# double125/MADTP

Hardware: AMD Instinct MI355X
Metric: images/sec forward, BLIP-base NLVR2 p=0.5 b64; pruned-token index match (higher is better)
Workload: dtype bf16

## Files before the change

### madtp_amd/csrc/attention.hip

```cpp
#include "common.h"
#include "internal.h"
#include <map>
#include <mutex>
#include <stdlib.h>

namespace {

struct AttnArgs {
    const char* q; const char* k; const char* v; char* out; const float* mask;
    float* colsum; float* p0; float* onorm;
    int B, H, Nq, Nk, ldq, ldk, ldv, ldo, nrt;
    float scale;
    const int* kvidx;
    const char* q2; const char* k2; const char* v2; char* out2; const float* mask2; int pair;
    const float* mask_qk; int ld_mqk;
    unsigned* hm_ws; int* hm_tick;
    int kvb;
    float* o_part;
    const int32_t* n_dev;
    int dev_q_only;
    int split_dim; int* range_flag;
};
#define ATTN_DEV_DIMS(a)                                   \
    if ((a).n_dev) {                                       \
// ... 373 lines not shown
#pragma unroll
        for (int t = 0; t < NT; ++t) {
            const int off = (16 * t + l16) * PITCH + g * 16;
            const f16x8 kh0 = *(const f16x8*)(K0 + off), kh1 = *(const f16x8*)(K0 + off + 64);
            const f16x8 kl0 = *(const f16x8*)(K1 + off), kl1 = *(const f16x8*)(K1 + off + 64);
            const f32x4 z = (f32x4){0.f, 0.f, 0.f, 0.f};
            f32x4 hi = __builtin_amdgcn_mfma_f32_16x16x32_f16(kh0, qh[0], z, 0, 0, 0);
            hi = __builtin_amdgcn_mfma_f32_16x16x32_f16(kh1, qh[1], hi, 0, 0, 0);
            f32x4 lo = __builtin_amdgcn_mfma_f32_16x16x32_f16(kh0, ql[0], z, 0, 0, 0);
            lo = __builtin_amdgcn_mfma_f32_16x16x32_f16(kh1, ql[1], lo, 0, 0, 0);
            lo = __builtin_amdgcn_mfma_f32_16x16x32_f16(kl0, qh[0], lo, 0, 0, 0);
            lo = __builtin_amdgcn_mfma_f32_16x16x32_f16(kl1, qh[1], lo, 0, 0, 0);
#pragma unroll
            for (int r = 0; r < 4; ++r) sc[t][r] = fmaf(lo[r], LO, hi[r]);
        }

        float m = -INFINITY;
#pragma unroll
        for (int t = 0; t < NT; ++t)
#pragma unroll
            for (int r = 0; r < 4; ++r) {
                const float v = __fadd_rn(__fmul_rn(sc[t][r], a.scale), mk[t][r]);
                sc[t][r] = v;
                m = fmaxf(m, v);
            }
        m = rows4_max(m);
        float sum = 0.f;
#pragma unroll
        for (int t = 0; t < NT; ++t)
#pragma unroll
            for (int r = 0; r < 4; ++r) {
                const float p = expf(sc[t][r] - m);
                sc[t][r] = p;
                sum += p;
            }
        sum = rows4_sum(sum);
#pragma unroll
        for (int t = 0; t < NT; ++t)
#pragma unroll
            for (int r = 0; r < 4; ++r) {
                const float p = sc[t][r] / sum;
                sc[t][r] = p;
                if constexpr (SCORES) pmax[t][r] = fmaxf(pmax[t][r], p);
            }
        if constexpr (SCORES) {
            if (i0 == 0 && l16 == 0) {
                float* dst = a.p0 + ((size_t)b * a.H + h) * a.Nk;
#pragma unroll
                for (int t = 0; t < NT; ++t)
#pragma unroll
                    for (int r = 0; r < 4; ++r) {
                        const int j = 16 * t + 4 * g + r;
                        if (j < a.Nk) dst[j] = sc[t][r];
                    }
            }
        }

        f32x4 oh[4], ol[4];
#pragma unroll
        for (int dt = 0; dt < 4; ++dt) { oh[dt] = (f32x4){0.f, 0.f, 0.f, 0.f}; ol[dt] = (f32x4){0.f, 0.f, 0.f, 0.f}; }
#pragma unroll
        for (int c = 0; c < NC; ++c) {
            const f32x4 t1 = (2 * c + 1 < NT) ? sc[2 * c + 1 < NT ? 2 * c + 1 : 0] : (f32x4){0.f, 0.f, 0.f, 0.f};
            u32x4 pp0, pp1;
            split_f16x8(sc[2 * c], t1, pp0, pp1);
            const f16x8 ph = __builtin_bit_cast(f16x8, pp0), pl = __builtin_bit_cast(f16x8, pp1);
            const int voff = (32 * c + 4 * g + (l16 >> 2)) * PITCH + 8 * (l16 & 3);
#pragma unroll
            for (int dt = 0; dt < 4; ++dt) {
                const bf16x8 vh = cat_bf16x4(lds_read_tr16(V0 + voff + dt * 32), lds_read_tr16(V0 + voff + 16 * PITCH + dt * 32));
                const bf16x8 vl = cat_bf16x4(lds_read_tr16(V1 + voff + dt * 32), lds_read_tr16(V1 + voff + 16 * PITCH + dt * 32));
                oh[dt] = __builtin_amdgcn_mfma_f32_16x16x32_f16(__builtin_bit_cast(f16x8, vh), ph, oh[dt], 0, 0, 0);
                ol[dt] = __builtin_amdgcn_mfma_f32_16x16x32_f16(__builtin_bit_cast(f16x8, vh), pl, ol[dt], 0, 0, 0);
                ol[dt] = __builtin_amdgcn_mfma_f32_16x16x32_f16(__builtin_bit_cast(f16x8, vl), ph, ol[dt], 0, 0, 0);
            }
        }

        {
            const int i = i0 + l16;
            f32x4 o[4];
            float n2 = 0.f;
#pragma unroll
            for (int dt = 0; dt < 4; ++dt)
#pragma unroll
                for (int r = 0; r < 4; ++r) {
                    o[dt][r] = fmaf(ol[dt][r], LO, oh[dt][r]);
                    n2 += o[dt][r] * o[dt][r];
                }
            if constexpr (SCORES) n2 = rows4_sum(n2);
            if (i < a.Nq) {
                if (a.split_dim) {
                    _Float16* prow = (_Float16*)a.out + ((size_t)b * a.Nq + i) * a.ldo + h * 64 + 4 * g;
                    bool bad = false;
#pragma unroll
                    for (int dt = 0; dt < 4; ++dt) {
                        f16x4 ph_, pl_;
                        split_f16x4(o[dt], ph_, pl_);
                        *(f16x4*)(prow + dt * 16) = ph_;
                        *(f16x4*)(prow + a.split_dim + dt * 16) = pl_;
                        bad |= f16_range_bad(o[dt]);
                    }
                    f16_range_raise(a.range_flag, bad);
                } else {
                    float* orow = (float*)(a.out + (((size_t)b * a.Nq + i) * a.ldo + h * 64) * 4) + 4 * g;
#pragma unroll
                    for (int dt = 0; dt < 4; ++dt) *(f32x4*)(orow + dt * 16) = o[dt];
                }
                if constexpr (SCORES)
                    if (g == 0) a.onorm[((size_t)b * a.H + h) * a.Nq + i] = sqrtf(n2);
            }
        }
    }

    if constexpr (SCORES) {
        if (gridDim.z == 2) {
            const size_t slot = ((size_t)b * gridDim.x + blockIdx.x) * 4 + wave;
            unsigned* mine = a.hm_ws + ((slot * 2 + blockIdx.z) * (2 * HM_MAX_NT)) * 64 + lane;
#pragma unroll
            for (int t = 0; t < NT; ++t)
#pragma unroll
                for (int r = 0; r < 4; ++r)
                    __hip_atomic_store(mine + (4 * t + r) * 64, __float_as_uint(pmax[t][r]), __ATOMIC_RELAXED, __HIP_MEMORY_SCOPE_AGENT);
            asm volatile("s_waitcnt vmcnt(0)" ::: "memory");
            int old = 0;
            if (lane == 0) old = __hip_atomic_fetch_add(a.hm_tick + slot, 1, __ATOMIC_RELAXED, __HIP_MEMORY_SCOPE_AGENT);
            old = __builtin_amdgcn_readfirstlane(old);
            if (old == 0) return;
            if (lane == 0) __hip_atomic_store(a.hm_tick + slot, 0, __ATOMIC_RELAXED, __HIP_MEMORY_SCOPE_AGENT);
            const unsigned* theirs = a.hm_ws + ((slot * 2 + (1 - blockIdx.z)) * (2 * HM_MAX_NT)) * 64 + lane;
#pragma unroll
            for (int t = 0; t < NT; ++t)
#pragma unroll
                for (int r = 0; r < 4; ++r)
                    pmax[t][r] = fmaxf(pmax[t][r], __uint_as_float(__hip_atomic_load(theirs + (4 * t + r) * 64, __ATOMIC_RELAXED,
                                                                                      __HIP_MEMORY_SCOPE_AGENT)));
        }
        if (active) {
            const int i = i0 + l16;
            const bool valid = i >= 1 && i < a.Nq;
            float* dst = a.colsum + ((size_t)b * a.nrt + rt) * a.Nk;
#pragma unroll
            for (int t = 0; t < NT; ++t)
#pragma unroll
                for (int r = 0; r < 4; ++r) {
                    const float v = row16_sum(valid ? pmax[t][r] : 0.f);
                    const int j = 16 * t + 4 * g + r;
                    if (l16 == 0 && j < a.Nk) dst[j] = v;
                }
        }
    }
}

#ifdef MADTP_TS_TIMING
__device__ long long g_attn_dbg[8];
#define AT_MARK(i) do { if (threadIdx.x == 0 && blockIdx.x == 0 && blockIdx.y == 0 && it == 2) { __builtin_amdgcn_s_waitcnt(0); g_attn_dbg[i] = wall_clock64(); } } while (0)
#else
#define AT_MARK(i)
#endif
template <int NT, bool SCORES, int HS, int RB = 1, bool F16 = false>
__global__ __launch_bounds__(256 * HS * RB, (HS == 1 && RB == 1) ? 2 : 1) void attn_bf16_kernel(AttnArgs a) {
    ATTN_DEV_DIMS(a)
    static_assert(HS == 1 || RB == 1, "head-parity split and two row blocks are alternatives");
    constexpr int NKP = NT * 16;
    constexpr int NC = (NT + 1) / 2;
    constexpr int VR = NC * 32;
    constexpr int STAGE = (NKP + VR) * 128;
    extern __shared__ __attribute__((aligned(16))) char smem[];

    const int tid = threadIdx.x, lane = tid & 63;
    const int wave8 = __builtin_amdgcn_readfirstlane(tid >> 6);
    const int wave = wave8 & 3;
    const int hp = HS == 2 ? wave8 >> 2 : 0;
    const int rb = RB == 2 ? wave8 >> 2 : 0;
    constexpr int NSW = 4 * RB;
    const int swave = RB == 2 ? wave8 : wave;
    char* const ring = smem + hp * 2 * STAGE;
    const int l16 = lane & 15, g = lane >> 4;
    int b = blockIdx.y;
    if (a.pair && b >= a.B) {
        b -= a.B;
        a.q = a.q2; a.k = a.k2; a.v = a.v2; a.out = a.out2; a.mask = a.mask2;
    }
    const int bkv = a.kvidx ? a.kvidx[b] : b;
    const int rt = (blockIdx.x * RB + rb) * 4 + wave;
    const int i0 = rt * 16;
    const bool active = i0 < a.Nq;
    const int irow = min(i0 + l16, a.Nq - 1);

    f32x4 pmax[NT];
    if constexpr (SCORES) {
#pragma unroll
        for (int t = 0; t < NT; ++t) pmax[t] = (f32x4){0.f, 0.f, 0.f, 0.f};
    }
    f32x4 mk[NT];
#pragma unroll
    for (int t = 0; t < NT; ++t)
#pragma unroll
        for (int r = 0; r < 4; ++r) {
            const int j = 16 * t + 4 * g + r;
            mk[t][r] = j < a.Nk ? (a.mask ? a.mask[(size_t)b * a.Nk + j] : 0.f) : -INFINITY;
            if (a.mask_qk && j < a.Nk) mk[t][r] += a.mask_qk[(size_t)irow * a.ld_mqk + j];
            mk[t][r] *= 1.44269504088896341f;
        }
    const float c2 = a.scale * 1.44269504088896341f;

    const int sub = lane >> 3, pos = lane & 7;
    constexpr int NDMA = ((NKP + VR) / 8 + NSW - 1) / NSW;
    const char* srcb[NDMA];
#pragma unroll
    for (int i = 0; i < NDMA; ++i) {
        const int grp = swave + NSW * i;
        const bool is_v = grp >= NKP / 8;
        int row = (is_v ? grp - NKP / 8 : grp) * 8 + sub;
        const int chunk = is_v ? (pos ^ (((row >> 1) & 3) << 1)) : (pos ^ (row & 7));
        row = row < a.Nk ? row : a.Nk - 1;
        srcb[i] = (is_v ? a.v + ((size_t)bkv * a.kvb + row) * a.ldv * 2 : a.k + ((size_t)bkv * a.kvb + row) * a.ldk * 2) + chunk * 16;
    }
    auto stage_head = [&](int h, int st) {
        char* base = ring + st * STAGE;
#pragma unroll
        for (int i = 0; i < NDMA; ++i) {
            const int grp = swave + NSW * i;
            if (grp < (NKP + VR) / 8)
                __builtin_amdgcn_global_load_lds(GLOBAL_PTR(srcb[i] + h * 128), LDS_PTR(base + grp * 1024), 16, 0, 0);
        }
    };
    const char* qbase = a.q + ((size_t)b * a.Nq + irow) * a.ldq * 2 + g * 16;
    auto load_q = [&](int h, bf16x8 (&qq)[2]) {
        const char* qp = qbase + h * 128;
        qq[0] = *(const bf16x8*)qp;
        qq[1] = *(const bf16x8*)(qp + 64);
    };
    int st = 0;
    const int hstep = gridDim.z * HS;
    const int hfirst = blockIdx.z * HS + hp;
    const int niter = (a.H - (int)blockIdx.z * HS + hstep - 1) / hstep;
    bf16x8 qn[2];
    if (hfirst < a.H) {
        stage_head(hfirst, 0);
        load_q(hfirst, qn);
    }
    for (int it = 0; it < niter; ++it, st ^= 1) {
        const int h = hfirst + it * hstep;
        bf16x8 q[2] = {qn[0], qn[1]};
        AT_MARK(0);
        __syncthreads();
        AT_MARK(1);
        if (h + hstep < a.H) {
            stage_head(h + hstep, st ^ 1);
            load_q(h + hstep, qn);
        }
        if (!active || h >= a.H) continue;
        AT_MARK(2);
        const char* Ks = ring + st * STAGE;
        const char* Vs = Ks + NKP * 128;

        f32x4 sc[NT];
#pragma unroll
        for (int t = 0; t < NT; ++t) {
            const int row = 16 * t + l16;
            const bf16x8 k0 = *(const bf16x8*)(Ks + row * 128 + (((0 + g) ^ (row & 7)) << 4));
            const bf16x8 k1 = *(const bf16x8*)(Ks + row * 128 + (((4 + g) ^ (row & 7)) << 4));
            f32x4 acc = (f32x4){0.f, 0.f, 0.f, 0.f};
            acc = mfma_lp<F16>(k0, q[0], acc, 0, 0, 0);
            sc[t] = mfma_lp<F16>(k1, q[1], acc, 0, 0, 0);
        }
        AT_MARK(3);
        float m = -INFINITY;
#pragma unroll
        for (int t = 0; t < NT; ++t)
#pragma unroll
            for (int r = 0; r < 4; ++r) {
                const float v = fmaf(sc[t][r], c2, mk[t][r]);
                sc[t][r] = v;
                m = fmaxf(m, v);
            }
        m = rows4_max(m);
        float sum = 0.f;
#pragma unroll
        for (int t = 0; t < NT; ++t)
#pragma unroll
            for (int r = 0; r < 4; ++r) {
                const float p = __builtin_amdgcn_exp2f(sc[t][r] - m);
                sc[t][r] = p;
                sum += p;
            }
        sum = rows4_sum(sum);
        const float inv = __builtin_amdgcn_rcpf(sum);
#pragma unroll
        for (int t = 0; t < NT; ++t) {
            sc[t] *= inv;
            if constexpr (SCORES) {
#pragma unroll
                for (int r = 0; r < 4; ++r) pmax[t][r] = fmaxf(pmax[t][r], sc[t][r]);
            }
        }
        if constexpr (SCORES) {
            if (i0 == 0) {
                if (l16 == 0) {
                    float* dst = a.p0 + ((size_t)b * a.H + h) * a.Nk;
#pragma unroll
                    for (int t = 0; t < NT; ++t)
#pragma unroll
                        for (int r = 0; r < 4; ++r) {
                            const int j = 16 * t + 4 * g + r;
                            if (j < a.Nk) dst[j] = sc[t][r];
                        }
                }
            }
        }
        AT_MARK(4);
        f32x4 o[4];
#pragma unroll
        for (int dt = 0; dt < 4; ++dt) o[dt] = (f32x4){0.f, 0.f, 0.f, 0.f};
#pragma unroll
        for (int c = 0; c < NC; ++c) {
            const f32x4 hi = (2 * c + 1 < NT) ? sc[2 * c + 1 < NT ? 2 * c + 1 : 0] : (f32x4){0.f, 0.f, 0.f, 0.f};
            const bf16x8 pa = pack_lp8<F16>(sc[2 * c], hi);
            const int vrow = 32 * c + 4 * g + (l16 >> 2);
            const int vkey = ((vrow >> 1) & 3) << 1;
            const char* vr = Vs + vrow * 128 + 8 * (l16 & 1);
#pragma unroll
            for (int dt = 0; dt < 4; ++dt) {
                const int p = ((2 * dt + ((l16 & 3) >> 1)) ^ vkey) << 4;
                const bf16x8 vb = cat_bf16x4(lds_read_tr16(vr + p), lds_read_tr16(vr + 16 * 128 + p));
                o[dt] = mfma_lp<F16>(vb, pa, o[dt], 0, 0, 0);
            }
        }
        AT_MARK(5);
        {
            const int i = i0 + l16;
            float n2 = 0.f;
#pragma unroll
            for (int dt = 0; dt < 4; ++dt)
#pragma unroll
                for (int r = 0; r < 4; ++r) n2 += o[dt][r] * o[dt][r];
            if constexpr (SCORES) {
                n2 = rows4_sum(n2);
            }
            if (i < a.Nq) {
                bf16_t* orow = (bf16_t*)(a.out + (((size_t)b * a.Nq + i) * a.ldo + h * 64) * 2) + 4 * g;
#pragma unroll
                for (int dt = 0; dt < 4; ++dt) *(bf16x4*)(orow + dt * 16) = pack_lp4<F16>(o[dt]);
                if constexpr (SCORES)
                    if (g == 0) a.onorm[((size_t)b * a.H + h) * a.Nq + i] = sqrtf(n2);
            }
        }
        AT_MARK(6);
    }

    if constexpr (SCORES && HS == 2) {
        f32x4* xch = (f32x4*)smem;
        __syncthreads();
        if (hp == 1)
#pragma unroll
            for (int t = 0; t < NT; ++t) xch[(wave * NT + t) * 64 + lane] = pmax[t];
        __syncthreads();
        if (hp == 1) return;
#pragma unroll
        for (int t = 0; t < NT; ++t) {
            const f32x4 o = xch[(wave * NT + t) * 64 + lane];
#pragma unroll
            for (int r = 0; r < 4; ++r) pmax[t][r] = fmaxf(pmax[t][r], o[r]);
        }
    }
    if constexpr (SCORES) {
        if (active) {
            const int i = i0 + l16;
            const bool valid = i >= 1 && i < a.Nq;
            float* dst = a.colsum + ((size_t)b * a.nrt + rt) * a.Nk;
#pragma unroll
            for (int t = 0; t < NT; ++t)
#pragma unroll
                for (int r = 0; r < 4; ++r) {
                    const float v = row16_sum(valid ? pmax[t][r] : 0.f);
                    const int j = 16 * t + 4 * g + r;
                    if (l16 == 0 && j < a.Nk) dst[j] = v;
                }
        }
    }
}

constexpr int SMALL_NW = 12;
template <bool F16>
__global__ __launch_bounds__(64 * SMALL_NW, 1) void attn_bf16_small_kernel(AttnArgs a) {
    __shared__ __attribute__((aligned(16))) char vbuf[SMALL_NW][32 * 128];
    __shared__ float pm[SMALL_NW][2][2][64][4];
    const int tid = threadIdx.x, lane = tid & 63;
    const int wave = __builtin_amdgcn_readfirstlane(tid >> 6);
    const int l16 = lane & 15, g = lane >> 4;
    const int b = blockIdx.x;
    const int N = a.Nk;
    char* Vs = vbuf[wave];
    f32x4 pmax[2][2];
#pragma unroll
    for (int rt = 0; rt < 2; ++rt)
#pragma unroll
        for (int t = 0; t < 2; ++t) pmax[rt][t] = (f32x4){0.f, 0.f, 0.f, 0.f};
    const int nrt = (N + 15) / 16;
    f32x4 mk[2];
#pragma unroll
    for (int t = 0; t < 2; ++t)
#pragma unroll
        for (int r = 0; r < 4; ++r) {
            const int j = 16 * t + 4 * g + r;
            mk[t][r] = (j < N ? (a.mask ? a.mask[(size_t)b * N + j] : 0.f) : -INFINITY) * 1.44269504088896341f;
        }
    const float c2 = a.scale * 1.44269504088896341f;

    for (int h = wave; h < a.H; h += SMALL_NW) {
        {
            const int sub = lane >> 3, pos = lane & 7;
#pragma unroll
            for (int grp = 0; grp < 4; ++grp) {
                int row = grp * 8 + sub;
                const int chunk = pos ^ (((row >> 1) & 3) << 1);
                row = row < N ? row : N - 1;
                *(bf16x8*)(Vs + grp * 1024 + lane * 16) =
                    *(const bf16x8*)(a.v + (((size_t)b * N + row) * a.ldv + h * 64) * 2 + chunk * 16);
            }
        }
        bf16x8 kf[2][2];
#pragma unroll
        for (int t = 0; t < 2; ++t) {
            const int j = min(16 * t + l16, N - 1);
            const char* kp = a.k + (((size_t)b * N + j) * a.ldk + h * 64) * 2 + g * 16;
            kf[t][0] = *(const bf16x8*)kp;
            kf[t][1] = *(const bf16x8*)(kp + 64);
        }
#pragma unroll
        for (int rt = 0; rt < 2; ++rt) {
            if (rt >= nrt) break;
            const int i0 = rt * 16;
            const int irow = min(i0 + l16, N - 1);
            const char* qp = a.q + (((size_t)b * N + irow) * a.ldq + h * 64) * 2 + g * 16;
            const bf16x8 q0 = *(const bf16x8*)qp, q1 = *(const bf16x8*)(qp + 64);
            f32x4 sc[2];
            float m = -INFINITY;
#pragma unroll
            for (int t = 0; t < 2; ++t) {
                f32x4 acc = (f32x4){0.f, 0.f, 0.f, 0.f};
                acc = mfma_lp<F16>(kf[t][0], q0, acc, 0, 0, 0);
                acc = mfma_lp<F16>(kf[t][1], q1, acc, 0, 0, 0);
#pragma unroll
                for (int r = 0; r < 4; ++r) {
                    const float v = fmaf(acc[r], c2, mk[t][r]);
                    acc[r] = v;
                    m = fmaxf(m, v);
                }
                sc[t] = acc;
            }
            m = rows4_max(m);
            float sum = 0.f;
#pragma unroll
            for (int t = 0; t < 2; ++t)
#pragma unroll
                for (int r = 0; r < 4; ++r) { sc[t][r] = __builtin_amdgcn_exp2f(sc[t][r] - m); sum += sc[t][r]; }
            sum = rows4_sum(sum);
            const float inv = __builtin_amdgcn_rcpf(sum);
#pragma unroll
            for (int t = 0; t < 2; ++t) {
                sc[t] *= inv;
#pragma unroll
                for (int r = 0; r < 4; ++r) pmax[rt][t][r] = fmaxf(pmax[rt][t][r], sc[t][r]);
            }
            if (i0 == 0) if (l16 == 0) {
                float* dst = a.p0 + ((size_t)b * a.H + h) * N;
#pragma unroll
                for (int t = 0; t < 2; ++t)
#pragma unroll
                    for (int r = 0; r < 4; ++r) {
                        const int j = 16 * t + 4 * g + r;
                        if (j < N) dst[j] = sc[t][r];
                    }
            }
            const bf16x8 pa = pack_lp8<F16>(sc[0], sc[1]);
            const int vrow = 4 * g + (l16 >> 2);
            const int vkey = ((vrow >> 1) & 3) << 1;
            const char* vr = Vs + vrow * 128 + 8 * (l16 & 1);
            f32x4 o[4];
            float n2 = 0.f;
#pragma unroll
            for (int dt = 0; dt < 4; ++dt) {
                const int p = ((2 * dt + ((l16 & 3) >> 1)) ^ vkey) << 4;
                const bf16x8 vb = cat_bf16x4(lds_read_tr16(vr + p), lds_read_tr16(vr + 16 * 128 + p));
                o[dt] = mfma_lp<F16>(vb, pa, (f32x4){0.f, 0.f, 0.f, 0.f}, 0, 0, 0);
#pragma unroll
                for (int r = 0; r < 4; ++r) n2 += o[dt][r] * o[dt][r];
            }
            n2 = rows4_sum(n2);
            const int i = i0 + l16;
            if (i < N) {
                bf16_t* orow = (bf16_t*)(a.out + (((size_t)b * N + i) * a.ldo + h * 64) * 2) + 4 * g;
#pragma unroll
                for (int dt = 0; dt < 4; ++dt) *(bf16x4*)(orow + dt * 16) = pack_lp4<F16>(o[dt]);
                if (g == 0) a.onorm[((size_t)b * a.H + h) * N + i] = sqrtf(n2);
            }
        }
    }
#pragma unroll
    for (int rt = 0; rt < 2; ++rt)
#pragma unroll
        for (int t = 0; t < 2; ++t)
#pragma unroll
            for (int r = 0; r < 4; ++r) pm[wave][rt][t][lane][r] = pmax[rt][t][r];
    __syncthreads();
    if (wave < nrt) {
        const int rt = wave, i = rt * 16 + l16;
        const bool valid = i >= 1 && i < N;
        float* dst = a.colsum + ((size_t)b * a.nrt + rt) * N;
#pragma unroll
        for (int t = 0; t < 2; ++t)
#pragma unroll
            for (int r = 0; r < 4; ++r) {
                float v = pm[0][rt][t][lane][r];
#pragma unroll
                for (int w = 1; w < SMALL_NW; ++w) v = fmaxf(v, pm[w][rt][t][lane][r]);
                v = row16_sum(valid ? v : 0.f);
                const int j = 16 * t + 4 * g + r;
                if (l16 == 0 && j < N) dst[j] = v;
            }
    }
}

template <int NT, bool SCORES, bool F16>
int launch_attn_bf16(const AttnArgs& a, hipStream_t s) {
    constexpr int NC = (NT + 1) / 2;
    constexpr int HS = (SCORES && NT <= 8) ? 2 : 1;
    constexpr int RB = (SCORES && NT > 8) ? 2 : 1;
    const size_t lds = (size_t)2 * HS * (NT * 16 + NC * 32) * 128;
    MADTP_ENSURE_MAX_LDS((attn_bf16_kernel<NT, SCORES, HS, RB, F16>), lds);
    int gz = 1;
    size_t lds_used = lds;
    if (!SCORES) {
        const int wgs = ((a.Nq + 63) / 64) * a.B;
        gz = wgs >= 512 ? 1 : a.H;
        if (gz == a.H) lds_used = lds / 2;
    }
    hipLaunchKernelGGL((attn_bf16_kernel<NT, SCORES, HS, RB, F16>), dim3((a.Nq + 64 * RB - 1) / (64 * RB), (!SCORES && a.pair) ? 2 * a.B : a.B, gz),
                       dim3(256 * HS * RB), lds_used, s, a);
    MADTP_LAUNCH_CHECK();
    return 0;
}

template <bool SCORES, bool F16 = false>
int dispatch_nt_bf16(const AttnArgs& a, hipStream_t s) {
    const int nt = (a.Nk + 15) / 16;
    if (nt <= 4) return launch_attn_bf16<4, SCORES, F16>(a, s);
    if (nt <= 6) return launch_attn_bf16<6, SCORES, F16>(a, s);
    if (nt <= 8) return launch_attn_bf16<8, SCORES, F16>(a, s);
    if (nt <= 10) return launch_attn_bf16<10, SCORES, F16>(a, s);
    if (nt <= 12) return launch_attn_bf16<12, SCORES, F16>(a, s);
    if (nt <= 13) return launch_attn_bf16<13, SCORES, F16>(a, s);
    if (nt <= 16) return launch_attn_bf16<16, SCORES, F16>(a, s);
    return MADTP_E_SHAPE;
}

template <typename T, int NCH, bool SCORES>
__global__ __launch_bounds__(256, 1) void attn_large_kernel(AttnArgs a) {
    constexpr int ESZ = sizeof(T);
    constexpr int RB = 64 * ESZ + 16;
    constexpr int CPR = 64 * ESZ / 16;
    constexpr int CK = 128;
    constexpr int NT = NCH * 8;
    extern __shared__ __attribute__((aligned(16))) char smem[];
    char* Ks = smem;
    char* Vs = smem + CK * RB;

    const int tid = threadIdx.x, lane = tid & 63, wave = tid >> 6;
    const int l16 = lane & 15, g = lane >> 4;
    const int b = blockIdx.y;
    const int bkv = a.kvidx ? a.kvidx[b] : b;
    const int rt = blockIdx.x * 4 + wave;
    const int i0 = rt * 16;
    const bool active = i0 < a.Nq;
    const int irow = min(i0 + l16, a.Nq - 1);

    f32x4 pmax[SCORES ? NT : 1];
    if constexpr (SCORES) {
#pragma unroll
        for (int t = 0; t < NT; ++t) pmax[t] = (f32x4){0.f, 0.f, 0.f, 0.f};
    }

    auto stage = [&](int h, int c, bool with_v) {
        for (int idx = tid; idx < CK * CPR; idx += 256) {
            const int row = idx / CPR, ch = idx % CPR, j = c * CK + row;
            uint4 kv = make_uint4(0, 0, 0, 0), vv = make_uint4(0, 0, 0, 0);
            if (j < a.Nk) {
                const size_t grow = (size_t)bkv * a.kvb + j;
                kv = *(const uint4*)(a.k + (grow * a.ldk + h * 64) * ESZ + ch * 16);
                if (with_v) vv = *(const uint4*)(a.v + (grow * a.ldv + h * 64) * ESZ + ch * 16);
            }
            *(uint4*)(Ks + row * RB + ch * 16) = kv;
            if (with_v) *(uint4*)(Vs + row * RB + ch * 16) = vv;
        }
    };
    auto scores = [&](int c, const f32x4 (&q)[4], f32x4 (&sc)[8]) {
#pragma unroll
        for (int t = 0; t < 8; ++t) sc[t] = (f32x4){0.f, 0.f, 0.f, 0.f};
#pragma unroll
        for (int s = 0; s < 4; ++s) {
            f32x4 kf[8];
#pragma unroll
            for (int t = 0; t < 8; ++t) kf[t] = load4<T>(Ks + (16 * t + l16) * RB + (4 * s + g) * 4 * ESZ);
#pragma unroll
            for (int e = 0; e < 4; ++e)
#pragma unroll
                for (int t = 0; t < 8; ++t) sc[t] = __builtin_amdgcn_mfma_f32_16x16x4f32(kf[t][e], q[s][e], sc[t], 0, 0, 0);
        }
#pragma unroll
        for (int t = 0; t < 8; ++t)
#pragma unroll
            for (int r = 0; r < 4; ++r) {
                const int j = c * CK + 16 * t + 4 * g + r;
                float v = sc[t][r] * a.scale;
                if (a.mask && j < a.Nk) v += a.mask[(size_t)b * a.Nk + j];
                sc[t][r] = j < a.Nk ? v : -INFINITY;
            }
    };

    for (int h = blockIdx.z; h < a.H; h += gridDim.z) {
        f32x4 q[4];
        {
            const char* qp = a.q + (((size_t)b * a.Nq + irow) * a.ldq + h * 64) * ESZ;
#pragma unroll
            for (int s = 0; s < 4; ++s) q[s] = load4<T>(qp + (4 * s + g) * 4 * ESZ);
        }
        float m = -INFINITY, l = 0.f;
        for (int c = 0; c < NCH; ++c) {
            if (c * CK >= a.Nk) break;
            __syncthreads();
            stage(h, c, false);
            __syncthreads();
            if (!active) continue;
            f32x4 sc[8];
            scores(c, q, sc);
            float cm = -INFINITY;
#pragma unroll
            for (int t = 0; t < 8; ++t)
#pragma unroll
                for (int r = 0; r < 4; ++r) cm = fmaxf(cm, sc[t][r]);
            cm = rows4_max(cm);
            const float mn = fmaxf(m, cm);
            float cs = 0.f;
#pragma unroll
            for (int t = 0; t < 8; ++t)
#pragma unroll
                for (int r = 0; r < 4; ++r) cs += expf(sc[t][r] - mn);
            cs = rows4_sum(cs);
            l = l * expf(m - mn) + cs;
            m = mn;
        }
        f32x4 o[4];
#pragma unroll
        for (int dt = 0; dt < 4; ++dt) o[dt] = (f32x4){0.f, 0.f, 0.f, 0.f};
#pragma unroll
        for (int c = 0; c < NCH; ++c) {
            if (c * CK < a.Nk) {
                __syncthreads();
                stage(h, c, true);
                __syncthreads();
                if (active) {
                    f32x4 sc[8];
                    scores(c, q, sc);
#pragma unroll
                    for (int t = 0; t < 8; ++t) {
#pragma unroll
                        for (int r = 0; r < 4; ++r) {
                            const float p = expf(sc[t][r] - m) / l;
                            sc[t][r] = p;
                            if constexpr (SCORES) pmax[c * 8 + t][r] = fmaxf(pmax[c * 8 + t][r], p);
                        }
                    }
                    if constexpr (SCORES) {
                        if (i0 + l16 == 0) {
                            float* dst = a.p0 + ((size_t)b * a.H + h) * a.Nk;
#pragma unroll
                            for (int t = 0; t < 8; ++t)
#pragma unroll
                                for (int r = 0; r < 4; ++r) {
                                    const int j = c * CK + 16 * t + 4 * g + r;
                                    if (j < a.Nk) dst[j] = sc[t][r];
                                }
// ... 906 lines not shown
}
int madtp_i_attention_mask(const void* q, const void* k, const void* v, void* out, const float* add_mask, float* colsum_part, float* p0,
                           float* onorm, int B, int H, int N, int ldq, int ldk, int ldv, int ldo, float scale, int io_dtype,
                           const int32_t* n_dev, void* stream) {
    if (N > 256) return MADTP_E_SHAPE;
    return madtp_i_attention_launch(q, k, v, nullptr, out, add_mask, nullptr, 0, colsum_part, p0, onorm, B, H, N, N, ldq, ldk, ldv, ldo, scale,
                                    io_dtype, 0, stream, n_dev);
}
int madtp_i_attention_cached(const void* q, const void* k, const void* v, int kv_block_rows, void* out, int B, int H, int Nq, int Nk,
                             int ldq, int ldk, int ldv, int ldo, float scale, int io_dtype, void* stream) {
    return madtp_i_attention_launch(q, k, v, nullptr, out, nullptr, nullptr, 0, nullptr, nullptr, nullptr, B, H, Nq, Nk, ldq, ldk, ldv, ldo, scale,
                                    io_dtype, 0, stream, nullptr, 0, kv_block_rows);
}
int madtp_i_attention_cross(const void* q, const void* k, const void* v, const int32_t* kv_batch_index, void* out, const float* add_mask,
                            int B, int H, int Nq_max, int Nk, int ldq, int ldk, int ldv, int ldo, float scale, int io_dtype,
                            const int32_t* nq_dev, void* stream) {
    if (Nk > 256 || Nq_max > 256) return MADTP_E_SHAPE;
    return madtp_i_attention_launch(q, k, v, kv_batch_index, out, add_mask, nullptr, 0, nullptr, nullptr, nullptr, B, H, Nq_max, Nk, ldq, ldk,
                                    ldv, ldo, scale, io_dtype, 0, stream, nq_dev, 1);
}

extern "C" int madtp_attention_indexed(const void* q, const void* k, const void* v, const int32_t* kv_batch_index, void* out,
                                       const float* add_mask, float* colsum_part, float* p0, float* onorm, int B, int H,
                                       int Nq, int Nk, int ldq, int ldk, int ldv, int ldo, float scale, int io_dtype,
                                       void* stream) {
    return madtp_i_attention_launch(q, k, v, kv_batch_index, out, add_mask, nullptr, 0, colsum_part, p0, onorm, B, H, Nq, Nk, ldq, ldk,
                                    ldv, ldo, scale, io_dtype, 0, stream);
}

extern "C" int madtp_attention_qk_mask(const void* q, const void* k, const void* v, void* out, const float* add_mask,
                                       const float* mask_qk, int ld_mask_qk, float* colsum_part, float* p0, float* onorm, int B,
                                       int H, int Nq, int Nk, int ldq, int ldk, int ldv, int ldo, float scale, int io_dtype,
                                       void* stream) {
    return madtp_i_attention_launch(q, k, v, nullptr, out, add_mask, mask_qk, ld_mask_qk, colsum_part, p0, onorm, B, H, Nq, Nk, ldq, ldk,
                                    ldv, ldo, scale, io_dtype, 0, stream);
}

bool madtp_internal_attn_f16s_enabled() {
    static const int f16s_env = env_int("MADTP_ATTN_F16S", 1);
    return f16s_env != 0;
}

int madtp_i_attention_launch(const void* q, const void* k, const void* v, const int32_t* kv_batch_index, void* out,
                             const float* add_mask, const float* mask_qk, int ld_mask_qk, float* colsum_part, float* p0,
                             float* onorm, int B, int H, int Nq, int Nk, int ldq, int ldk, int ldv, int ldo, float scale,
                             int io_dtype, int split_req, void* stream, const int32_t* n_dev, int dev_q_only, int kv_block_rows) {
    if (!q || !k || !v || !out || B <= 0 || H <= 0 || Nq <= 0 || Nk <= 0) return MADTP_E_BADARG;
    if (mask_qk && (ld_mask_qk < Nk || Nk > 256)) return MADTP_E_SHAPE;
    if (split_req < 0) split_req = 0;
    if (kv_block_rows && (kv_block_rows < Nk || Nk > 256 || colsum_part)) return MADTP_E_SHAPE;
    if (kv_batch_index && colsum_part) return MADTP_E_BADARG;
    if (io_dtype != MADTP_F32 && io_dtype != MADTP_BF16 && io_dtype != MADTP_F16S && io_dtype != MADTP_F16) return MADTP_E_DTYPE;
    bool f16s = io_dtype == MADTP_F16S;
    const bool f16 = io_dtype == MADTP_F16;
    int split_dim = 0;
    if (f16s) {
        f16s = madtp_internal_attn_f16s_enabled();
        io_dtype = MADTP_F32;
        split_dim = f16s ? split_req : 0;
        if (split_req && !f16s) return MADTP_E_BADARG;
    } else if (split_req) {
        return MADTP_E_BADARG;
    }
    if (colsum_part && (!p0 || !onorm || Nq != Nk)) return MADTP_E_BADARG;
    const int esz = (io_dtype == MADTP_BF16 || f16) ? 2 : 4;
    if (!aligned16(q) || !aligned16(k) || !aligned16(v) || (ldq * esz) % 16 || (ldk * esz) % 16 || (ldv * esz) % 16)
        return MADTP_E_ALIGN;
    if (Nk > 1024) return MADTP_E_SHAPE;
    AttnArgs a;
    a.q = (const char*)q; a.k = (const char*)k; a.v = (const char*)v; a.out = (char*)out; a.mask = add_mask;
    a.colsum = colsum_part; a.p0 = p0; a.onorm = onorm;
    a.B = B; a.H = H; a.Nq = Nq; a.Nk = Nk; a.ldq = ldq; a.ldk = ldk; a.ldv = ldv; a.ldo = ldo;
    a.nrt = (Nq + 15) / 16;
    a.scale = scale;
    a.kvidx = kv_batch_index;
    a.pair = 0; a.q2 = a.k2 = a.v2 = nullptr; a.out2 = nullptr; a.mask2 = nullptr; a.hm_ws = nullptr; a.hm_tick = nullptr; a.o_part = nullptr;
    a.mask_qk = mask_qk; a.ld_mqk = ld_mask_qk;
    a.n_dev = n_dev; a.dev_q_only = dev_q_only;
    a.kvb = kv_block_rows ? kv_block_rows : Nk;
    a.split_dim = split_dim; a.range_flag = split_dim ? madtp_internal_range_flag() : nullptr;
    hipStream_t s = (hipStream_t)stream;
    const bool scores = colsum_part != nullptr;
    if (split_dim) {
        if ((ldo % 4) || (split_dim % 4) || ((uintptr_t)out & 7)) return MADTP_E_ALIGN;
        if (Nk > 256) return scores ? dispatch_large_f16s<true>(a, s) : dispatch_large_f16s<false>(a, s);
        return scores ? dispatch_nt_f16s<true>(a, s) : dispatch_nt_f16s<false>(a, s);
    }
    if (Nk > 256) {
        if (f16s && (ldo * 4) % 16 == 0 && aligned16(out))
            return scores ? dispatch_large_f16s<true>(a, s) : dispatch_large_f16s<false>(a, s);
        if (io_dtype == MADTP_F32) return scores ? dispatch_large<float, true>(a, s) : dispatch_large<float, false>(a, s);
        static const int large_env = env_int("MADTP_ATTN_LARGE_F32", 0);
        if (f16) return scores ? dispatch_bf16_large<true, true>(a, s) : dispatch_bf16_large<false, true>(a, s);
        if (large_env) return scores ? dispatch_large<bf16_t, true>(a, s) : dispatch_large<bf16_t, false>(a, s);
        return scores ? dispatch_bf16_large<true>(a, s) : dispatch_bf16_large<false>(a, s);
    }
    if (f16s && (ldo * 4) % 16 == 0 && aligned16(out))
        return scores ? dispatch_nt_f16s<true>(a, s) : dispatch_nt_f16s<false>(a, s);
    if (io_dtype == MADTP_F32) return scores ? dispatch_nt<float, true>(a, s) : dispatch_nt<float, false>(a, s);
    if ((ldk * 2) % 16 || (ldv * 2) % 16) return MADTP_E_ALIGN;
    if (scores && Nk <= 32 && !mask_qk && !n_dev) {
        if (f16) hipLaunchKernelGGL(attn_bf16_small_kernel<true>, dim3(B), dim3(64 * SMALL_NW), 0, s, a);
        else hipLaunchKernelGGL(attn_bf16_small_kernel<false>, dim3(B), dim3(64 * SMALL_NW), 0, s, a);
        MADTP_LAUNCH_CHECK();
        return 0;
    }
    if (f16) return scores ? dispatch_nt_bf16<true, true>(a, s) : dispatch_nt_bf16<false, true>(a, s);
    return scores ? dispatch_nt_bf16<true>(a, s) : dispatch_nt_bf16<false>(a, s);
}

extern "C" int madtp_attention_pair(const void* q0, const void* q1, const void* k0, const void* k1, const void* v0, const void* v1,
                                    const int32_t* kv_batch_index, void* out0, void* out1, const float* add_mask0,
                                    const float* add_mask1, int B, int H, int Nq, int Nk, int ldq, int ldk, int ldv, int ldo,
                                    float scale, int io_dtype, void* stream) {
    return madtp_i_attention_pair(q0, q1, k0, k1, v0, v1, kv_batch_index, out0, out1, add_mask0, add_mask1, B, H, Nq, Nk, ldq, ldk, ldv,
                                  ldo, scale, io_dtype, 0, nullptr, stream);
}
int madtp_i_attention_pair(const void* q0, const void* q1, const void* k0, const void* k1, const void* v0, const void* v1,
                           const int32_t* kv_batch_index, void* out0, void* out1, const float* add_mask0, const float* add_mask1, int B,
                           int H, int Nq, int Nk, int ldq, int ldk, int ldv, int ldo, float scale, int io_dtype, int split_dim,
                           const int32_t* nq_dev, void* stream) {
    if (nq_dev && (Nk > 256 || Nq > 256)) return MADTP_E_SHAPE;
    if (!q0 || !q1 || !k0 || !k1 || !v0 || !v1 || !out0 || !out1 || B <= 0 || H <= 0 || Nq <= 0 || Nk <= 0) return MADTP_E_BADARG;
    static const int pair_env = env_int("MADTP_ATTN_PAIR", 1);
    const bool one = pair_env && (io_dtype == MADTP_BF16 || io_dtype == MADTP_F16) && Nk <= 256 && (!add_mask0) == (!add_mask1) && aligned16(q0) &&
                     aligned16(q1) && aligned16(k0) && aligned16(k1) && aligned16(v0) && aligned16(v1) && (ldq * 2) % 16 == 0 &&
                     (ldk * 2) % 16 == 0 && (ldv * 2) % 16 == 0;
    if (!one) {
        const int rc = madtp_i_attention_launch(q0, k0, v0, kv_batch_index, out0, add_mask0, nullptr, 0, nullptr, nullptr, nullptr, B, H, Nq, Nk,
                                                ldq, ldk, ldv, ldo, scale, io_dtype, split_dim, stream, nq_dev, nq_dev ? 1 : 0);
        if (rc) return rc;
        return madtp_i_attention_launch(q1, k1, v1, kv_batch_index, out1, add_mask1, nullptr, 0, nullptr, nullptr, nullptr, B, H, Nq, Nk, ldq,
                                        ldk, ldv, ldo, scale, io_dtype, split_dim, stream, nq_dev, nq_dev ? 1 : 0);
    }
    if (split_dim) return MADTP_E_BADARG;
    AttnArgs a;
    a.q = (const char*)q0; a.k = (const char*)k0; a.v = (const char*)v0; a.out = (char*)out0; a.mask = add_mask0;
    a.q2 = (const char*)q1; a.k2 = (const char*)k1; a.v2 = (const char*)v1; a.out2 = (char*)out1; a.mask2 = add_mask1;
    a.pair = 1;
    a.mask_qk = nullptr; a.ld_mqk = 0; a.hm_ws = nullptr; a.hm_tick = nullptr; a.n_dev = nq_dev; a.dev_q_only = 1; a.o_part = nullptr;
    a.colsum = nullptr; a.p0 = nullptr; a.onorm = nullptr; a.split_dim = 0; a.range_flag = nullptr;
    a.B = B; a.H = H; a.Nq = Nq; a.Nk = Nk; a.ldq = ldq; a.ldk = ldk; a.ldv = ldv; a.ldo = ldo;
    a.kvb = Nk;
    a.nrt = (Nq + 15) / 16;
    a.scale = scale;
    a.kvidx = kv_batch_index;
    if (io_dtype == MADTP_F16) return dispatch_nt_bf16<false, true>(a, (hipStream_t)stream);
    return dispatch_nt_bf16<false>(a, (hipStream_t)stream);
}

#ifdef MADTP_TS_TIMING
extern "C" int madtp_debug_read_attn_ts(long long* out) {
    hipDeviceSynchronize();
    return (int)hipMemcpyFromSymbol(out, HIP_SYMBOL(g_attn_dbg), sizeof(long long) * 8);
}
#endif
```

Measured before the change: 26400.

## Split small score-attention heads across two workgroups with global max exchange

```diff
diff --git a/madtp_amd/csrc/attention.hip b/madtp_amd/csrc/attention.hip
--- a/madtp_amd/csrc/attention.hip
+++ b/madtp_amd/csrc/attention.hip
@@ -549,15 +549,33 @@
 }
 
 #ifdef MADTP_TS_TIMING
-__device__ long long g_attn_dbg[8];
-#define AT_MARK(i) do { if (threadIdx.x == 0 && blockIdx.x == 0 && blockIdx.y == 0 && it == 2) { __builtin_amdgcn_s_waitcnt(0); g_attn_dbg[i] = wall_clock64(); } } while (0)
+__device__ long long g_attn_dbg[32];
+#define AT_MARK_IF(c, i) do { if (threadIdx.x == 0 && blockIdx.x == 0 && blockIdx.y == 0 && (c)) { __builtin_amdgcn_s_waitcnt(0); g_attn_dbg[(i) + 16 * (blockIdx.z & 1)] = wall_clock64(); } } while (0)
+#define AT_MARK(i) AT_MARK_IF(it == 2, i)
+#define AT_MARK_K(i) AT_MARK_IF(true, i)
 #else
+#define AT_MARK_IF(c, i)
 #define AT_MARK(i)
+#define AT_MARK_K(i)
 #endif
-template <int NT, bool SCORES, int HS, int RB = 1, bool F16 = false>
-__global__ __launch_bounds__(256 * HS * RB, (HS == 1 && RB == 1) ? 2 : 1) void attn_bf16_kernel(AttnArgs a) {
+template <int CTRL>
+__device__ __forceinline__ float dpp_row(float v) {
+    return __builtin_bit_cast(float, __builtin_amdgcn_mov_dpp(__builtin_bit_cast(int, v), CTRL, 0xf, 0xf, true));
+}
+__device__ __forceinline__ float row16_sum_lane0(float v) {
+    v += dpp_row<0x128>(v);
+    v += dpp_row<0x104>(v);
+    v += dpp_row<0x4e>(v);
+    v += dpp_row<0xb1>(v);
+    return v;
+}
+
+template <int NT, bool SCORES, int HS, int RB = 1, bool F16 = false, int RT = 4, bool HC = false>
+__global__ __launch_bounds__(64 * RT * HS * RB, (HS == 1 && RB == 1) ? 2 : 1) void attn_bf16_kernel(AttnArgs a) {
+    AT_MARK_K(8);
     ATTN_DEV_DIMS(a)
     static_assert(HS == 1 || RB == 1, "head-parity split and two row blocks are alternatives");
+    static_assert(HC ? (SCORES && HS == 2 && RT >= NT) : RT == 4, "the head cut holds all row tiles of a sample in one workgroup");
     constexpr int NKP = NT * 16;
     constexpr int NC = (NT + 1) / 2;
     constexpr int VR = NC * 32;
@@ -566,10 +584,10 @@
 
     const int tid = threadIdx.x, lane = tid & 63;
     const int wave8 = __builtin_amdgcn_readfirstlane(tid >> 6);
-    const int wave = wave8 & 3;
-    const int hp = HS == 2 ? wave8 >> 2 : 0;
-    const int rb = RB == 2 ? wave8 >> 2 : 0;
-    constexpr int NSW = 4 * RB;
+    const int wave = wave8 % RT;
+    const int hp = HS == 2 ? wave8 / RT : 0;
+    const int rb = RB == 2 ? wave8 / RT : 0;
+    constexpr int NSW = RT * RB;
     const int swave = RB == 2 ? wave8 : wave;
     char* const ring = smem + hp * 2 * STAGE;
     const int l16 = lane & 15, g = lane >> 4;
@@ -579,7 +597,7 @@
         a.q = a.q2; a.k = a.k2; a.v = a.v2; a.out = a.out2; a.mask = a.mask2;
     }
     const int bkv = a.kvidx ? a.kvidx[b] : b;
-    const int rt = (blockIdx.x * RB + rb) * 4 + wave;
+    const int rt = (blockIdx.x * RB + rb) * RT + wave;
     const int i0 = rt * 16;
     const bool active = i0 < a.Nq;
     const int irow = min(i0 + l16, a.Nq - 1);
@@ -589,16 +607,6 @@
 #pragma unroll
         for (int t = 0; t < NT; ++t) pmax[t] = (f32x4){0.f, 0.f, 0.f, 0.f};
     }
-    f32x4 mk[NT];
-#pragma unroll
-    for (int t = 0; t < NT; ++t)
-#pragma unroll
-        for (int r = 0; r < 4; ++r) {
-            const int j = 16 * t + 4 * g + r;
-            mk[t][r] = j < a.Nk ? (a.mask ? a.mask[(size_t)b * a.Nk + j] : 0.f) : -INFINITY;
-            if (a.mask_qk && j < a.Nk) mk[t][r] += a.mask_qk[(size_t)irow * a.ld_mqk + j];
-            mk[t][r] *= 1.44269504088896341f;
-        }
     const float c2 = a.scale * 1.44269504088896341f;
 
     const int sub = lane >> 3, pos = lane & 7;
@@ -637,12 +645,30 @@
         stage_head(hfirst, 0);
         load_q(hfirst, qn);
     }
+    f32x4 mk[NT];
+    if (!a.mask && !a.mask_qk) {
+#pragma unroll
+        for (int t = 0; t < NT; ++t)
+#pragma unroll
+            for (int r = 0; r < 4; ++r) mk[t][r] = 16 * t + 4 * g + r < a.Nk ? 0.f : -INFINITY;
+    } else {
+#pragma unroll
+        for (int t = 0; t < NT; ++t)
+#pragma unroll
+            for (int r = 0; r < 4; ++r) {
+                const int j = 16 * t + 4 * g + r;
+                mk[t][r] = j < a.Nk ? (a.mask ? a.mask[(size_t)b * a.Nk + j] : 0.f) : -INFINITY;
+                if (a.mask_qk && j < a.Nk) mk[t][r] += a.mask_qk[(size_t)irow * a.ld_mqk + j];
+                mk[t][r] *= 1.44269504088896341f;
+            }
+    }
     for (int it = 0; it < niter; ++it, st ^= 1) {
         const int h = hfirst + it * hstep;
         bf16x8 q[2] = {qn[0], qn[1]};
         AT_MARK(0);
         __syncthreads();
         AT_MARK(1);
+        AT_MARK_IF(it == 0, 9);
         if (h + hstep < a.H) {
             stage_head(h + hstep, st ^ 1);
             load_q(h + hstep, qn);
@@ -746,6 +772,7 @@
         AT_MARK(6);
     }
 
+    AT_MARK_K(10);
     if constexpr (SCORES && HS == 2) {
         f32x4* xch = (f32x4*)smem;
         __syncthreads();
@@ -760,22 +787,67 @@
 #pragma unroll
             for (int r = 0; r < 4; ++r) pmax[t][r] = fmaxf(pmax[t][r], o[r]);
         }
+    }
+    if constexpr (HC) {
+        if (!active) return;
+        AT_MARK_K(11);
+        const size_t slot = (size_t)b * RT + wave;
+        unsigned* mine = a.hm_ws + ((slot * 2 + blockIdx.z) * (2 * HM_MAX_NT)) * 64 + lane;
+#pragma unroll
+        for (int t = 0; t < NT; ++t)
+#pragma unroll
+            for (int r = 0; r < 4; ++r)
+                __hip_atomic_store(mine + (4 * t + r) * 64, __float_as_uint(pmax[t][r]), __ATOMIC_RELAXED, __HIP_MEMORY_SCOPE_AGENT);
+        asm volatile("s_waitcnt vmcnt(0)" ::: "memory");
+        AT_MARK_K(12);
+        int old = 0;
+        if (lane == 0) old = __hip_atomic_fetch_add(a.hm_tick + slot, 1, __ATOMIC_RELAXED, __HIP_MEMORY_SCOPE_AGENT);
+        old = __builtin_amdgcn_readfirstlane(old);
+        AT_MARK_K(13);
+        if (old == 0) return;
+        __builtin_amdgcn_fence(__ATOMIC_ACQUIRE, "wavefront");
+        if (lane == 0) __hip_atomic_store(a.hm_tick + slot, 0, __ATOMIC_RELAXED, __HIP_MEMORY_SCOPE_AGENT);
+        const unsigned* theirs = a.hm_ws + ((slot * 2 + (1 - blockIdx.z)) * (2 * HM_MAX_NT)) * 64 + lane;
+#pragma unroll
+        for (int t = 0; t < NT; ++t)
+#pragma unroll
+            for (int r = 0; r < 4; ++r)
+                pmax[t][r] = fmaxf(pmax[t][r], __uint_as_float(__hip_atomic_load(theirs + (4 * t + r) * 64, __ATOMIC_RELAXED,
+                                                                                  __HIP_MEMORY_SCOPE_AGENT)));
+        AT_MARK_K(14);
     }
     if constexpr (SCORES) {
         if (active) {
             const int i = i0 + l16;
             const bool valid = i >= 1 && i < a.Nq;
             float* dst = a.colsum + ((size_t)b * a.nrt + rt) * a.Nk;
-#pragma unroll
-            for (int t = 0; t < NT; ++t)
-#pragma unroll
-                for (int r = 0; r < 4; ++r) {
-                    const float v = row16_sum(valid ? pmax[t][r] : 0.f);
-                    const int j = 16 * t + 4 * g + r;
-                    if (l16 == 0 && j < a.Nk) dst[j] = v;
-                }
-        }
-    }
+            if constexpr (NT <= 13) {
+#pragma unroll
+                for (int t = 0; t < NT; ++t)
+#pragma unroll
+                    for (int r = 0; r < 4; ++r) pmax[t][r] = row16_sum_lane0(valid ? pmax[t][r] : 0.f);
+                if (l16 == 0) {
+#pragma unroll
+                    for (int t = 0; t < NT; ++t)
+#pragma unroll
+                        for (int r = 0; r < 4; ++r) {
+                            const int j = 16 * t + 4 * g + r;
+                            if (j < a.Nk) dst[j] = pmax[t][r];
+                        }
+                }
+            } else {
+#pragma unroll
+                for (int t = 0; t < NT; ++t)
+#pragma unroll
+                    for (int r = 0; r < 4; ++r) {
+                        const float v = row16_sum(valid ? pmax[t][r] : 0.f);
+                        const int j = 16 * t + 4 * g + r;
+                        if (l16 == 0 && j < a.Nk) dst[j] = v;
+                    }
+            }
+        }
+    }
+    AT_MARK_K(15);
 }
 
 constexpr int SMALL_NW = 12;
@@ -926,6 +998,20 @@
     constexpr int HS = (SCORES && NT <= 8) ? 2 : 1;
     constexpr int RB = (SCORES && NT > 8) ? 2 : 1;
     const size_t lds = (size_t)2 * HS * (NT * 16 + NC * 32) * 128;
+    if constexpr (SCORES && NT <= 6) {
+        constexpr int RT = NT <= 4 ? 4 : 6;
+        static_assert(4 * NT <= 2 * HM_MAX_NT && RT >= NT, "exchange rows per wave");
+        static const int headcut_env = env_int("MADTP_ATTN_HEADCUT", 1);
+        HmWorkspace hw;
+        if (headcut_env && !a.n_dev && !a.pair && a.Nq <= 16 * RT && a.Nk <= 16 * NT && a.B <= HM_MAX_WGS * 4 / RT && hm_workspace(s, hw)) {
+            AttnArgs ac = a;
+            ac.hm_ws = hw.ws; ac.hm_tick = hw.tick;
+            MADTP_ENSURE_MAX_LDS((attn_bf16_kernel<NT, true, 2, 1, F16, RT, true>), lds);
+            hipLaunchKernelGGL((attn_bf16_kernel<NT, true, 2, 1, F16, RT, true>), dim3(1, a.B, 2), dim3(64 * RT * 2), lds, s, ac);
+            MADTP_LAUNCH_CHECK();
+            return 0;
+        }
+    }
     MADTP_ENSURE_MAX_LDS((attn_bf16_kernel<NT, SCORES, HS, RB, F16>), lds);
     int gz = 1;
     size_t lds_used = lds;
@@ -2138,6 +2224,6 @@
 #ifdef MADTP_TS_TIMING
 extern "C" int madtp_debug_read_attn_ts(long long* out) {
     hipDeviceSynchronize();
-    return (int)hipMemcpyFromSymbol(out, HIP_SYMBOL(g_attn_dbg), sizeof(long long) * 8);
+    return (int)hipMemcpyFromSymbol(out, HIP_SYMBOL(g_attn_dbg), sizeof(long long) * 32);
 }
 #endif
```

New measurement: 26660 (median of 4 runs). 1.01x the previous value.
